# limanling/clip-event

Measured on AMD Instinct MI355X. Metric: image-text pairs/sec/GPU, ViT-B/32 224px x 77-tok, global-batch contrastive, higher is better.
Workload: dtype bf16; 1 GPU; ViT-B/32 224px x 77-tok, bf16 operands, per-GPU batch 256, K=1, InfoNCE only, full train step (fwd+bwd+clip_grad_norm+Adam), random-init weights; global_batch=256, parallelism=dp1, captions=SOT + U[8,75] random ids + EOT, zero-padded to 77 (SURVEY 8(d) c2), text_rows=live tokens SOT..EOT only: 54.8% of B*77 rows (identical results, see DESIGN.md), fresh_captions_every_step=True, alignment=False, cu_hog=0, nt_pgrid=256, full=False

## Files before the change

### clip_event_amd/csrc/attention.hip

```cpp
#include <map>
#include <mutex>

#include <type_traits>

#include "common.hpp"
#include "../../include/clip_event_hip.h"

namespace {

constexpr int HD = 64;
constexpr int ROW = 160;

typedef __attribute__((address_space(3))) s16x4 lds_s16x4;
typedef __attribute__((ext_vector_type(8))) short s16x8;

__device__ __forceinline__ bf16x8 tr_pair(const char* p0, const char* p1) {
    s16x4 lo = __builtin_amdgcn_ds_read_tr16_b64_v4i16((lds_s16x4*)p0);
    s16x4 hi = __builtin_amdgcn_ds_read_tr16_b64_v4i16((lds_s16x4*)p1);
    s16x8 v = {lo[0], lo[1], lo[2], lo[3], hi[0], hi[1], hi[2], hi[3]};
    return __builtin_bit_cast(bf16x8, v);
}

__device__ __forceinline__ bf16x8 pack8(const f32x4& a, const f32x4& b) {
    u32x4 v = {pack_bf2(a[0], a[1]), pack_bf2(a[2], a[3]), pack_bf2(b[0], b[1]), pack_bf2(b[2], b[3])};
// ... 113 lines not shown
                *reinterpret_cast<u32x2*>(orow + ct * 16) = pk;
            }
            if (g == 0) lse[((long)b * H + h) * Lmax + i] = mx + __logf(sum);
        }
    }
}

template <int T>
__global__ __launch_bounds__(512) void attn_bwd_kernel(const bf16_t* __restrict__ qkv, long ld,
                                                       const bf16_t* __restrict__ o, long ldo,
                                                       const bf16_t* __restrict__ dout, long lddo,
                                                       const float* __restrict__ lse, bf16_t* __restrict__ dqkv,
                                                       long lddq, float* __restrict__ bias_grad,
                                                       const int* __restrict__ cu, int Lmax, int H, int D,
                                                       int causal, float scale) {
    extern __shared__ __attribute__((aligned(16))) char smem[];
    constexpr int Lp = T * 16;
    constexpr int PROW = Lp * 2 + 32;
    char* sA = smem;
    char* sB = sA + Lp * ROW;
    char* sP = sB + Lp * ROW;
    char* sDS = sP + Lp * PROW;
    auto csum = [&](int i) __attribute__((always_inline)) -> float* { return reinterpret_cast<float*>(sP + (i >> 3) * PROW + Lp * 2 + (i & 7) * 4); };
    const int tid = threadIdx.x, lane = tid & 63;
    const int wave = __builtin_amdgcn_readfirstlane(tid >> 6), nw = blockDim.x >> 6;
    const int b = blockIdx.x / H, h = blockIdx.x - b * H;
    const long row0 = cu ? (long)cu[b] : (long)b * Lmax;
    const int L = cu ? min(cu[b + 1] - cu[b], Lmax) : Lmax;
    if (L <= 0) return;
    const int Tl = ((L + 31) >> 5) << 1;
    const int Ll = Tl * 16;
    const bf16_t* base = qkv + row0 * ld + h * HD;
    const bf16_t* dob = dout + row0 * lddo + h * HD;
    const bf16_t* ob = o + row0 * ldo + h * HD;
    bf16_t* dbase = dqkv + row0 * lddq + h * HD;

    for (int i = tid; i < 192; i += blockDim.x) *csum(i) = 0.f;
    const int li = lane & 15, g = lane >> 4;
    u32x4 rK[2], rV[2], rQ[2], rD[2];
#pragma unroll
    for (int c = 0; c < 2; ++c) {
        const int idx = tid + c * blockDim.x;
        const int r = idx >> 3, ch = idx & 7;
        const u32x4 z = {0u, 0u, 0u, 0u};
        rK[c] = z; rV[c] = z; rQ[c] = z; rD[c] = z;
        if (idx < Ll * 8 && r < L) {
            rK[c] = *reinterpret_cast<const u32x4*>(base + D + (long)r * ld + ch * 8);
            rV[c] = *reinterpret_cast<const u32x4*>(base + 2 * D + (long)r * ld + ch * 8);
            rQ[c] = *reinterpret_cast<const u32x4*>(base + (long)r * ld + ch * 8);
            rD[c] = *reinterpret_cast<const u32x4*>(dob + (long)r * lddo + ch * 8);
        }
    }
    const int strip = wave;
    const bool has_strip = strip < Tl;
    const int i = strip * 16 + li;
    const bool iok = has_strip && i < L;
    const int iq = min(i, L - 1);
    float dl = 0.f, lsei = 0.f;
    bf16x8 qf[2], df[2];
    if (has_strip) {
        const u32x4* pd = reinterpret_cast<const u32x4*>(dob + (long)iq * lddo + g * 16);
        const u32x4* po = reinterpret_cast<const u32x4*>(ob + (long)iq * ldo + g * 16);
#pragma unroll
        for (int v = 0; v < 2; ++v) {
            u32x4 a = pd[v], c = po[v];
#pragma unroll
            for (int e = 0; e < 4; ++e) dl += bf_lo(a[e]) * bf_lo(c[e]) + bf_hi(a[e]) * bf_hi(c[e]);
        }
        lsei = lse[((long)b * H + h) * Lmax + iq];
#pragma unroll
        for (int ks = 0; ks < 2; ++ks) {
            qf[ks] = *reinterpret_cast<const bf16x8*>(base + (long)iq * ld + ks * 32 + g * 8);
            df[ks] = *reinterpret_cast<const bf16x8*>(dob + (long)iq * lddo + ks * 32 + g * 8);
        }
    }
#pragma unroll
    for (int c = 0; c < 2; ++c) {
        const int idx = tid + c * blockDim.x;
        if (idx < Ll * 8) {
            *reinterpret_cast<u32x4*>(sA + (idx >> 3) * ROW + (idx & 7) * 16) = rK[c];
            *reinterpret_cast<u32x4*>(sB + (idx >> 3) * ROW + (idx & 7) * 16) = rV[c];
        }
    }
    __syncthreads();
    dl += __shfl_xor(dl, 16, 64);
    dl += __shfl_xor(dl, 32, 64);

    if (has_strip) {
        f32x4 p[T], ds[T];
#pragma unroll
        for (int t = 0; t < T; ++t) {
            p[t] = f32x4{0.f, 0.f, 0.f, 0.f};
            ds[t] = f32x4{0.f, 0.f, 0.f, 0.f};
            if (t >= Tl) continue;
#pragma unroll
            for (int ks = 0; ks < 2; ++ks) {
                bf16x8 kf = *reinterpret_cast<const bf16x8*>(sA + (t * 16 + li) * ROW + (ks * 4 + g) * 16);
                bf16x8 vf = *reinterpret_cast<const bf16x8*>(sB + (t * 16 + li) * ROW + (ks * 4 + g) * 16);
                p[t] = __builtin_amdgcn_mfma_f32_16x16x32_bf16(kf, qf[ks], p[t], 0, 0, 0);
                ds[t] = __builtin_amdgcn_mfma_f32_16x16x32_bf16(vf, df[ks], ds[t], 0, 0, 0);
            }
#pragma unroll
            for (int r = 0; r < 4; ++r) {
                const int j = t * 16 + g * 4 + r;
                const bool ok = iok && (j < L) && (!causal || j <= i);
                const float pv = ok ? __expf(p[t][r] * scale - lsei) : 0.f;
                p[t][r] = pv;
                ds[t][r] = pv * (ds[t][r] - dl) * scale;
            }
            u32x2 pk = {pack_bf2(p[t][0], p[t][1]), pack_bf2(p[t][2], p[t][3])};
            u32x2 dk = {pack_bf2(ds[t][0], ds[t][1]), pack_bf2(ds[t][2], ds[t][3])};
            *reinterpret_cast<u32x2*>(sP + i * PROW + (t * 16 + g * 4) * 2) = pk;
            *reinterpret_cast<u32x2*>(sDS + i * PROW + (t * 16 + g * 4) * 2) = dk;
        }
        f32x4 acc[4];
#pragma unroll
        for (int ct = 0; ct < 4; ++ct) acc[ct] = f32x4{0.f, 0.f, 0.f, 0.f};
#pragma unroll
        for (int sidx = 0; sidx < T / 2; ++sidx) {
            if (2 * sidx >= Tl) continue;
            bf16x8 sf = pack8(ds[2 * sidx], ds[2 * sidx + 1]);
            const char* krow = sA + (32 * sidx + 4 * g + (li >> 2)) * ROW + (4 * (li & 3)) * 2;
#pragma unroll
            for (int ct = 0; ct < 4; ++ct) {
                bf16x8 kf = tr_pair(krow + ct * 32, krow + ct * 32 + 16 * ROW);
                acc[ct] = __builtin_amdgcn_mfma_f32_16x16x32_bf16(kf, sf, acc[ct], 0, 0, 0);
            }
        }
        if (iok) {
            bf16_t* qrow = dbase + (long)i * lddq + 4 * g;
#pragma unroll
            for (int ct = 0; ct < 4; ++ct) {
                u32x2 pk = {pack_bf2(acc[ct][0], acc[ct][1]), pack_bf2(acc[ct][2], acc[ct][3])};
                *reinterpret_cast<u32x2*>(qrow + ct * 16) = pk;
            }
        }
        if (bias_grad) {
            float vals[16];
#pragma unroll
            for (int ct = 0; ct < 4; ++ct)
#pragma unroll
                for (int r = 0; r < 4; ++r) vals[ct * 4 + r] = acc[ct][r];
// ... 37 lines not shown
                av[ct] = __builtin_amdgcn_mfma_f32_16x16x32_bf16(dof, pf, av[ct], 0, 0, 0);
                ak[ct] = __builtin_amdgcn_mfma_f32_16x16x32_bf16(qf, sf, ak[ct], 0, 0, 0);
            }
        }
        if (j < L) {
            bf16_t* krow = dbase + (long)j * lddq + D + 4 * g;
            bf16_t* vrow = dbase + (long)j * lddq + 2 * D + 4 * g;
#pragma unroll
            for (int ct = 0; ct < 4; ++ct) {
                u32x2 pk = {pack_bf2(ak[ct][0], ak[ct][1]), pack_bf2(ak[ct][2], ak[ct][3])};
                u32x2 pv = {pack_bf2(av[ct][0], av[ct][1]), pack_bf2(av[ct][2], av[ct][3])};
                *reinterpret_cast<u32x2*>(krow + ct * 16) = pk;
                *reinterpret_cast<u32x2*>(vrow + ct * 16) = pv;
            }
        }
        if (bias_grad) {
            float vk[16], vv[16];
#pragma unroll
            for (int ct = 0; ct < 4; ++ct)
#pragma unroll
                for (int r = 0; r < 4; ++r) {
                    vk[ct * 4 + r] = ak[ct][r];
                    vv[ct * 4 + r] = av[ct][r];
                }
            const float tk = row16_colsum(vk, li), tv = row16_colsum(vv, li);
            const int k = row16_colsum_index(li);
            atomicAdd(csum(64 + (k >> 2) * 16 + 4 * g + (k & 3)), tk);
            atomicAdd(csum(128 + (k >> 2) * 16 + 4 * g + (k & 3)), tv);
        }
    }
    if (bias_grad) {
        __syncthreads();
        for (int i = tid; i < 192; i += blockDim.x) atomicAdd(bias_grad + (i >> 6) * D + h * HD + (i & 63), *csum(i));
    }
}

constexpr int LB = 64;
constexpr int LPROW = LB * 2 + 32;

__device__ __forceinline__ void stage_block(char* dst, const bf16_t* src, long ld, int row0, int L, int tid) {
#pragma unroll
    for (int c = 0; c < 2; ++c) {
        const int idx = tid + c * 256;
        const int r = idx >> 3, ch = idx & 7;
        u32x4 v = {0u, 0u, 0u, 0u};
        if (row0 + r < L) v = *reinterpret_cast<const u32x4*>(src + (long)(row0 + r) * ld + ch * 8);
        *reinterpret_cast<u32x4*>(dst + r * ROW + ch * 16) = v;
    }
}

struct BlockRegs { u32x4 v[2]; };
__device__ __forceinline__ BlockRegs load_block(const bf16_t* src, long ld, int row0, int L, int tid) {
    BlockRegs b;
#pragma unroll
    for (int c = 0; c < 2; ++c) {
        const int idx = tid + c * 256;
        const int r = idx >> 3, ch = idx & 7;
        b.v[c] = u32x4{0u, 0u, 0u, 0u};
        if (row0 + r < L) b.v[c] = *reinterpret_cast<const u32x4*>(src + (long)(row0 + r) * ld + ch * 8);
    }
    return b;
}
__device__ __forceinline__ void store_block(char* dst, const BlockRegs& b, int tid) {
#pragma unroll
    for (int c = 0; c < 2; ++c) {
        const int idx = tid + c * 256;
// ... 562 lines not shown
        if (nk == 1)
            hipLaunchKernelGGL(attn_bwd_long_dkv_kernel<1>, grid1, dim3(256), 0, sl, (const bf16_t*)qkv, ld, (const bf16_t*)o, ldo,
                               (const bf16_t*)dout, lddo, lse, (bf16_t*)dqkv, lddq, bias_grad, delta, L, H, D, causal, 0.125f, attn_xcd_order());
        else
            hipLaunchKernelGGL(attn_bwd_long_dkv_kernel<2>, grid2, dim3(256), 0, sl, (const bf16_t*)qkv, ld, (const bf16_t*)o, ldo,
                               (const bf16_t*)dout, lddo, lse, (bf16_t*)dqkv, lddq, bias_grad, delta, L, H, D, causal, 0.125f, attn_xcd_order());
        CE_LAUNCH_CHECK();
        return 0;
    }
    const int T = tiles_for(L);
    const int Lp = T * 16;
    int nw = T;
    if (nw > 8) nw = 8;
    const size_t lds = 2 * (size_t)Lp * ROW + 2 * (size_t)Lp * (Lp * 2 + 32);
    const float scale = 0.125f;
    hipStream_t s = (hipStream_t)stream;
    CeProfScope prof(CE_PROF_ATTN_BWD, 10.0 * B * H * (double)L * L * HD, 2.0 * (double)B * L * (8.0 * D), s);
#define CALL(TT)                                                                                                   \
    do {                                                                                                           \
        static std::once_flag attr;                                                                                \
        std::call_once(attr, [] {                                                                                  \
            hipFuncSetAttribute(reinterpret_cast<const void*>(attn_bwd_kernel<TT>),                                \
                                hipFuncAttributeMaxDynamicSharedMemorySize, 160 * 1024);                           \
        });                                                                                                        \
        hipLaunchKernelGGL(attn_bwd_kernel<TT>, dim3(B * H), dim3(64 * nw), lds, s, (const bf16_t*)qkv, ld,        \
                           (const bf16_t*)o, ldo, (const bf16_t*)dout, lddo, lse, (bf16_t*)dqkv, lddq, bias_grad, cu_seqlens, L, \
                           H, D, causal, scale);                                                                           \
    } while (0)
    ATTN_DISPATCH(T, CALL);
#undef CALL
    CE_LAUNCH_CHECK();
    return 0;
}
```

### clip_event_amd/csrc/tower.cpp

```cpp
#include <hip/hip_runtime.h>
#include <stdlib.h>

#include <map>
#include <mutex>

#include "common.hpp"
#include "tn_plan.hpp"
#include "../../include/clip_event_hip.h"

namespace {

constexpr int WG_MAX_BLOCKS = TN_GROUP_MAX_BLOCKS;
constexpr int WG_SETS = WG_MAX_BLOCKS + 1;
constexpr int LNP_RING = 8;

struct Carver {
    char* base;
    size_t off = 0;
    explicit Carver(void* b) : base(reinterpret_cast<char*>(b)) {}
    template <typename T>
    T* take(size_t n) {
        off = (off + 255) & ~size_t(255);
        T* p = base ? reinterpret_cast<T*>(base + off) : nullptr;
        off += n * sizeof(T);
// ... 96 lines not shown
    CE_CHECK_ARG(rows > 0 && (long)rows <= (long)batch * d->tokens, "tower: rows=%d outside 1..batch*tokens", rows);
    CE_CHECK_ARG(cu || rows == batch * d->tokens, "tower: a dense batch has batch*tokens rows (got %d)", rows);
    return 0;
}

int check_desc(const ce_tower_desc* d, int batch) {
    CE_CHECK_ARG(d && d->blocks, "tower: null descriptor");
    CE_CHECK_ARG(d->layers > 0 && d->layers <= Layout::MAX_LAYERS, "tower: layers=%d out of range", d->layers);
    CE_CHECK_ARG(d->width == d->heads * 64, "tower: width %d != heads %d * 64", d->width, d->heads);
    CE_CHECK_ARG(d->tokens > 0 && d->tokens <= 4096, "tower: tokens=%d unsupported (1..4096)", d->tokens);
    CE_CHECK_ARG(batch > 0, "tower: empty batch");
    CE_CHECK_ARG(d->stream16 == 0 || d->stream16 == 1, "tower: stream16=%d (0: fp32 residual stream, 1: fp16)", d->stream16);
    return 0;
}

#define TRY(call)            \
    do {                     \
        int rc__ = (call);   \
        if (rc__ != 0) return rc__; \
    } while (0)

int linear(bool use8, const Layout& L, const void*& q8_of, const void* A, long lda, const void* W, const void* W8, const float* S8, int M,
           int N, int K, int epi, const float* bias, const void* resid, long ldr, void* out, long ldo, void* out2,
           long ldo2, const void* aux, long ldaux, void* stream) {
    if (use8 && W8 && S8 && K % 128 == 0 && K <= 4096) {
        if (q8_of != A || lda != K) TRY(ce_quant_rows_fp8(A, lda, L.q8, K, L.q8s, M, K, stream));
        q8_of = nullptr;
        return ce_gemm_nt_fp8(L.q8, K, L.q8s, W8, K, S8, M, N, K, epi, bias, resid, ldr, out, ldo, out2, ldo2, aux, ldaux,
                              stream);
    }
    return ce_gemm_nt(A, lda, W, K, M, N, K, epi, bias, resid, ldr, out, ldo, out2, ldo2, aux, ldaux, stream);
}

int forward_run(const ce_tower_desc* d, int batch, int rows, const int* cu_seqlens, const void* x0, Layout& L, void* x_out,
                const int* sel_rows, bool infer, void* stream) {
    const int M = rows, w = d->width;
    const bool f8 = (d->fp8 & 1) != 0;
    const int ST = d->stream16 ? CE_T_F16 : CE_T_F32;
    const int EPI_RESID = d->stream16 ? CE_EPI_BIAS_RESID_F16 : CE_EPI_BIAS_RESID_F32;
    const int EPI_FC = infer ? CE_EPI_BIAS_QGELU_BF16 : CE_EPI_BIAS_GELU;
    const long esz = d->stream16 ? 2 : 4;
    const void* x = x0;
    const void* q8_of = nullptr;
    const bool lnq = f8 && w % 128 == 0 && w <= 4096;
    for (int l = 0; l < d->layers; ++l) {
        const ce_block_params& p = d->blocks[l];
        BlockStash& s = L.blk[l];
        void* xo = (l + 1 < d->layers) ? s.x_out : x_out;
        TRY(ce_layernorm_fwd_q8(x, ST, w, nullptr, p.ln1_w, p.ln1_b, s.h1, CE_T_BF16, w, s.mean1, s.rstd1, M, w, 1e-5f,
                                lnq ? L.q8 : nullptr, w, L.q8s, stream));
        if (lnq) q8_of = s.h1;
        TRY(linear(f8, L, q8_of, s.h1, w, p.w_qkv, p.w8_qkv, p.s8_qkv, M, 3 * w, w, CE_EPI_BIAS_BF16, p.b_qkv, nullptr, 0, s.qkv, 3 * w, nullptr, 0,
                       nullptr, 0, stream));
        TRY(ce_attention_fwd(s.qkv, 3 * w, s.o, w, s.lse, cu_seqlens, batch, d->tokens, d->heads, d->causal, stream));
        if (sel_rows && l + 1 == d->layers) {
            const int Bn = batch;
            TRY(ce_copy_rows(s.o, w * 2L, sel_rows, L.os, w * 2L, nullptr, Bn, w * 2, stream));
            TRY(ce_copy_rows(x, w * esz, sel_rows, L.xs_in, w * esz, nullptr, Bn, (int)(w * esz), stream));
            TRY(linear(f8, L, q8_of, L.os, w, p.w_out, p.w8_out, p.s8_out, Bn, w, w, EPI_RESID, p.b_out, L.xs_in, w, L.xs_mid, w, nullptr,
                           0, nullptr, 0, stream));
            TRY(ce_layernorm_fwd_t(L.xs_mid, ST, w, nullptr, p.ln2_w, p.ln2_b, L.h2s, CE_T_BF16, w, L.means, L.rstds, Bn, w, 1e-5f, stream));
            TRY(linear(f8, L, q8_of, L.h2s, w, p.w_fc, p.w8_fc, p.s8_fc, Bn, 4 * w, w, EPI_FC, p.b_fc, nullptr, 0, infer ? L.gs : L.as, 4 * w,
                           infer ? nullptr : L.gs, infer ? 0 : 4 * w, nullptr, 0, stream));
            TRY(linear(f8, L, q8_of, L.gs, 4 * w, p.w_proj, p.w8_proj, p.s8_proj, Bn, w, 4 * w, EPI_RESID, p.b_proj, L.xs_mid, w, x_out, w,
                           nullptr, 0, nullptr, 0, stream));
            break;
        }
        TRY(linear(f8, L, q8_of, s.o, w, p.w_out, p.w8_out, p.s8_out, M, w, w, EPI_RESID, p.b_out, x, w, s.x_mid, w, nullptr, 0, nullptr,
                       0, stream));
        TRY(ce_layernorm_fwd_q8(s.x_mid, ST, w, nullptr, p.ln2_w, p.ln2_b, s.h2, CE_T_BF16, w, s.mean2, s.rstd2, M, w, 1e-5f,
                                lnq ? L.q8 : nullptr, w, L.q8s, stream));
        if (lnq) q8_of = s.h2;
        TRY(linear(f8, L, q8_of, s.h2, w, p.w_fc, p.w8_fc, p.s8_fc, M, 4 * w, w, EPI_FC, p.b_fc, nullptr, 0, infer ? s.g : s.a, 4 * w,
                       infer ? nullptr : s.g, infer ? 0 : 4 * w, nullptr, 0, stream));
        TRY(linear(f8, L, q8_of, s.g, 4 * w, p.w_proj, p.w8_proj, p.s8_proj, M, w, 4 * w, EPI_RESID, p.b_proj, s.x_mid, w, xo, w,
                       nullptr, 0, nullptr, 0, stream));
        x = xo;
    }
    return 0;
}

}

extern "C" size_t ce_tower_workspace_bytes(const ce_tower_desc* d, int batch) {
    if (check_desc(d, batch) != 0) return 0;
    Layout L;
    carve(d, batch, (size_t)batch * d->tokens, nullptr, L);
    return L.bytes;
}

// ... 90 lines not shown
    } pend;
    auto queue = [&](const void* P, long ldp, const void* Q, long ldq, int Nn, int Kk, float* out, long ldo) {
        const int i = pend.count++;
        pend.P[i] = P; pend.ldp[i] = ldp; pend.Q[i] = Q; pend.ldq[i] = ldq;
        pend.Nn[i] = Nn; pend.Kk[i] = Kk; pend.out[i] = out; pend.ldo[i] = ldo;
    };
    auto flush = [&]() -> int {
        if (pend.count == 0) return 0;
        const int rc = ce_gemm_tn_grouped_ex(pend.count, pend.P, pend.ldp, pend.Q, pend.ldq, M, pend.Nn, pend.Kk, pend.out,
                                             pend.ldo, 0, d->wgrad_overwrite, stream);
        pend.count = 0;
        pend.blocks = 0;
        return rc;
    };
    int top = layer_hi;
    if (layer_hi < last) {
    } else if (sel_rows) {
        CE_CHECK_ARG(dx_sel, "ce_tower_backward: pruned mode needs dx_sel");
        const int l = top, Bn = batch, q = l % WG_SETS;
        const ce_block_params& p = d->blocks[l];
        BlockStash& s = L.blk[l];
        const void* x_in = (l == 0) ? x0 : L.blk[l - 1].x_out;
        TRY(ce_cast_bf16(dx_sel, L.dxbs, (long)Bn * w, stream));
        TRY(linear(b8, L, q8_of, L.dxbs, w, p.wt_proj, p.wt8_proj, p.st8_proj, Bn, 4 * w, w, CE_EPI_GELUGRAD_BF16, nullptr, nullptr, 0, L.das, 4 * w, nullptr,
                       0, L.as, 4 * w, stream));
        TRY(ce_colsum_bf16(L.dxbs, w, p.g_b_proj, Bn, w, stream));
        TRY(linear(b8, L, q8_of, L.das, 4 * w, p.wt_fc, p.wt8_fc, p.st8_fc, Bn, w, 4 * w, CE_EPI_BF16, nullptr, nullptr, 0, L.dhs, w, nullptr, 0,
                       nullptr, 0, stream));
        TRY(ce_colsum_bf16(L.das, 4 * w, p.g_b_fc, Bn, 4 * w, stream));
        TRY(ce_layernorm_bwd_t(L.dhs, CE_T_BF16, w, L.xs_mid, ST, w, nullptr, L.means, L.rstds, p.ln2_w, dx_sel, CE_T_F32, L.dxs_mid,
                               ST, w, L.dxb2s, w, p.g_ln2_w, p.g_ln2_b, p.g_b_out, GS, Bn, w, stream));
        TRY(linear(b8, L, q8_of, L.dxb2s, w, p.wt_out, p.wt8_out, p.st8_out, Bn, w, w, CE_EPI_BF16, nullptr, nullptr, 0, L.dos, w, nullptr, 0, nullptr, 0,
                       stream));
        TRY(ce_scatter_rows_zero(L.dos, w * 2L, L.d_o, w * 2L, sel_rows, Bn, M, w * 2, stream));
        TRY(ce_attention_bwd(s.qkv, 3 * w, s.o, w, L.d_o, w, s.lse, L.dqkv[q], 3 * w, p.g_b_qkv, cu_seqlens, batch, d->tokens, d->heads,
                             d->causal, stream));
        {
            const void* P[3] = {L.dxbs, L.das, L.dxb2s};
            const long ldp[3] = {w, 4L * w, w};
            const void* Q[3] = {L.gs, L.h2s, L.os};
            const long ldq[3] = {4L * w, w, w};
            const int Nn[3] = {w, 4 * w, w};
            const int Kk[3] = {4 * w, w, w};
            float* out[3] = {p.g_w_proj, p.g_w_fc, p.g_w_out};
            const long ldo[3] = {4L * w, w, w};
            TRY(ce_gemm_tn_grouped_ex(3, P, ldp, Q, ldq, Bn, Nn, Kk, out, ldo, 0, d->wgrad_overwrite, stream));
        }
        queue(L.dqkv[q], 3L * w, s.h1, w, 3 * w, w, p.g_w_qkv, w);
        TRY(linear(b8, L, q8_of, L.dqkv[q], 3 * w, p.wt_qkv, p.wt8_qkv, p.st8_qkv, M, w, 3 * w, CE_EPI_BF16, nullptr, nullptr, 0, L.dh, w, nullptr, 0,
                       nullptr, 0, stream));
        TRY(ce_scatter_rows_zero(L.dxs_mid, w * esz, dx, w * esz, sel_rows, Bn, M, (int)(w * esz), stream));
        TRY(ce_layernorm_bwd_t(L.dh, CE_T_BF16, w, x_in, ST, w, nullptr, s.mean1, s.rstd1, p.ln1_w, dx, ST, dx, ST, w,
                               L.dxb[(l + WG_SETS - 1) % WG_SETS], w, p.g_ln1_w, p.g_ln1_b,
                               (l > 0) ? d->blocks[l - 1].g_b_proj : nullptr, GS, M, w, stream));
        top = l - 1;
    } else {
        if (d->stream16) TRY(ce_cast_scaled(dx, ST, L.dxb[top % WG_SETS], CE_T_BF16, GS, 1, (long)M * w, stream));
        else TRY(ce_cast_bf16(reinterpret_cast<const float*>(dx), L.dxb[top % WG_SETS], (long)M * w, stream));
    }
    plan_cuts(top, layer_lo, pend.count > 0 ? 3 * tn_problem_tiles(M, w, w) : 0);
    for (int l = top; l >= layer_lo; --l) {
        const ce_block_params& p = d->blocks[l];
        BlockStash& s = L.blk[l];
        const int q = l % WG_SETS;
        bf16_t *dxb_a = L.dxb[q], *dxb_b = L.dxb2[q], *da = L.da[q], *dqkv = L.dqkv[q];
        const void* x_in = (l == 0) ? x0 : L.blk[l - 1].x_out;
        TRY(linear(b8, L, q8_of, dxb_a, w, p.wt_proj, p.wt8_proj, p.st8_proj, M, 4 * w, w, CE_EPI_GELUGRAD_BF16, nullptr, nullptr, 0, da, 4 * w, p.g_b_fc,
                       4 * w, s.a, 4 * w, stream));
        if (l == last) TRY(ce_colsum_bf16(dxb_a, w, p.g_b_proj, M, w, stream));
// ... 31 lines not shown
```

### clip_event_amd/ops.py

```python
from __future__ import annotations

from typing import Optional

import torch

from . import _lib as L
from ._lib import check, lib, ptr, stream


def _rows(t: torch.Tensor) -> int:
    return t.shape[0]


def _nt_tail(epilogue, bias, resid, out, out2, ldo2, aux):
    return (epilogue, ptr(bias), ptr(resid), resid.stride(0) if resid is not None else 0, ptr(out), out.stride(0), ptr(out2),
            ldo2, ptr(aux), aux.stride(0) if aux is not None else 0, stream())


def gemm_nt(a: torch.Tensor, b: torch.Tensor, epilogue: int, *, bias=None, resid=None, out=None, out2=None,
            aux=None, M: Optional[int] = None) -> torch.Tensor:
    assert a.dtype == torch.bfloat16 and b.dtype == torch.bfloat16 and a.is_cuda and b.is_cuda
    M = a.shape[0] if M is None else M
    K = a.shape[1]
    N = b.shape[0]
# ... 80 lines not shown
    return buf[:1]


def cast_scaled(x: torch.Tensor, dtype, scale: torch.Tensor, divide: bool = False):
    y = torch.empty_like(x, dtype=dtype)
    check(lib().ce_cast_scaled(ptr(x), _TYPE[x.dtype], ptr(y), _TYPE[dtype], ptr(scale), 1 if divide else 0,
                               x.numel(), stream()), "ce_cast_scaled")
    return y


def cast_t(x: torch.Tensor, dtype, mul: float = 1.0):
    y = torch.empty_like(x, dtype=dtype)
    check(lib().ce_cast_t(ptr(x), _TYPE[x.dtype], ptr(y), _TYPE[dtype], mul, x.numel(), stream()),
          "ce_cast_t")
    return y


def attention_fwd(qkv: torch.Tensor, B: int, L: int, H: int, causal: bool, cu_seqlens=None):
    assert qkv.dtype == torch.bfloat16
    o = torch.empty(qkv.shape[0], H * 64, device=qkv.device, dtype=torch.bfloat16)
    lse = torch.empty(B * H * L, device=qkv.device, dtype=torch.float32)
    check(lib().ce_attention_fwd(ptr(qkv), qkv.stride(0), ptr(o), o.stride(0), ptr(lse),
                                 ptr(cu_seqlens), B, L, H, 1 if causal else 0, stream()),
          "ce_attention_fwd")
    return o, lse


def attention_bwd(qkv, o, dout, lse, B: int, L: int, H: int, causal: bool, bias_grad=None, cu_seqlens=None):
    dqkv = torch.empty_like(qkv)
    check(lib().ce_attention_bwd(ptr(qkv), qkv.stride(0), ptr(o), o.stride(0), ptr(dout),
                                 dout.stride(0), ptr(lse), ptr(dqkv), dqkv.stride(0), ptr(bias_grad),
                                 ptr(cu_seqlens), B, L, H, 1 if causal else 0, stream()),
          "ce_attention_bwd")
    return dqkv


def probe_mfma(shape: int, a_frags: torch.Tensor, b_frags: torch.Tensor) -> torch.Tensor:
    out = torch.empty(64, 4 if shape == 16 else 16, device=a_frags.device, dtype=torch.float32)
    check(lib().ce_probe_mfma(shape, ptr(a_frags), ptr(b_frags), ptr(out), stream()), "ce_probe_mfma")
    return out


def probe_tr16(image: torch.Tensor, byte_off: torch.Tensor) -> torch.Tensor:
    out = torch.empty(64, 4, device=image.device, dtype=torch.int16)
    check(lib().ce_probe_tr16(ptr(image), image.numel(), ptr(byte_off), ptr(out), stream()), "ce_probe_tr16")
    return out


def quant_rows_fp8(x: torch.Tensor):
    assert x.dtype == torch.bfloat16 and x.is_cuda and x.stride(1) == 1
    M, K = x.shape
    q = torch.empty(M, K, dtype=torch.uint8, device=x.device)
    scale = torch.empty(M, dtype=torch.float32, device=x.device)
    check(lib().ce_quant_rows_fp8(ptr(x), x.stride(0), ptr(q), K, ptr(scale), M, K, stream()),
          "ce_quant_rows_fp8")
    return q, scale


def gemm_nt_fp8(a8, sa, b8, sb, epilogue: int, *, bias=None, resid=None, aux=None, colsum=None):
    M, K = a8.shape
    N = b8.shape[0]
    f32_out = epilogue == L.EPI_BIAS_RESID_F32
    out = torch.empty(M, N, device=a8.device, dtype=torch.float32 if f32_out else torch.bfloat16)
    out2 = torch.empty_like(out) if epilogue == L.EPI_BIAS_GELU else colsum
    ldo2 = out2.stride(0) if epilogue == L.EPI_BIAS_GELU else 0
    check(lib().ce_gemm_nt_fp8(ptr(a8), a8.stride(0), ptr(sa), ptr(b8), b8.stride(0), ptr(sb), M, N, K,
# ... 47 lines not shown
```

### include/clip_event_hip.h

```cpp
#ifndef CLIP_EVENT_HIP_H
#define CLIP_EVENT_HIP_H

#include <stddef.h>
#include <stdint.h>

#ifdef __cplusplus
extern "C" {
#endif

const char* ce_last_error(void);
int ce_version(void);

enum {
    CE_EPI_BF16 = 0,
    CE_EPI_F32 = 1,
    CE_EPI_BIAS_BF16 = 2,
    CE_EPI_BIAS_F32 = 3,
    CE_EPI_BIAS_RESID_F32 = 4,
    CE_EPI_BIAS_GELU = 5,
    CE_EPI_GELUGRAD_BF16 = 6,
    CE_EPI_BIAS_RESID_F16 = 7,
    CE_EPI_BIAS_QGELU_BF16 = 8
};

// ... 46 lines not shown
int ce_layernorm_bwd(const void* dy, long lddy, int dy_f32, const float* x, long ldx, const int* rows,
                     const float* mean, const float* rstd, const float* w, const float* dx_in, float* dx_out,
                     long lddx, void* dxb, long lddxb, float* dw, float* db, float* dxsum, int M, int D,
                     void* stream);
int ce_layernorm_bwd_t(const void* dy, int dy_type, long lddy, const void* x, int x_type, long ldx, const int* rows,
                       const float* mean, const float* rstd, const float* w, const void* dx_in, int dxin_type,
                       void* dx_out, int dx_type, long lddx, void* dxb, long lddxb, float* dw, float* db, float* dxsum,
                       const float* gscale, int M, int D, void* stream);

int ce_layernorm_bwd_q8(const void* dy, int dy_type, long lddy, const void* x, int x_type, long ldx, const int* rows,
                        const float* mean, const float* rstd, const float* w, const void* dx_in, int dxin_type,
                        void* dx_out, int dx_type, long lddx, void* dxb, long lddxb, float* dw, float* db, float* dxsum,
                        const float* gscale, int M, int D, void* q8, long ldq, float* qscale, void* stream);

int ce_layernorm_bwd_blocks(int M, int D);
int ce_layernorm_bwd_partials(const void* dy, int dy_type, long lddy, const void* x, int x_type, long ldx, const int* rows,
                              const float* mean, const float* rstd, const float* w, const void* dx_in, int dxin_type,
                              void* dx_out, int dx_type, long lddx, void* dxb, long lddxb, int want_dxsum,
                              const float* gscale, int M, int D, void* q8, long ldq, float* qscale, float* partials,
                              void* stream);
#define CE_LN_FOLD_MAX 64
typedef struct ce_ln_fold_job {
    const float* partials;
    float *dw, *db, *dxsum;
    int blocks, D;
} ce_ln_fold_job;
int ce_layernorm_fold(const ce_ln_fold_job* jobs , int njobs, void* stream);

int ce_attention_fwd(const void* qkv, long ld, void* o, long ldo, float* lse, const int* cu_seqlens, int B, int L,
                     int H, int causal, void* stream);
int ce_attention_bwd(const void* qkv, long ld, const void* o, long ldo, const void* dout, long lddo,
                     const float* lse, void* dqkv, long lddq, float* bias_grad, const int* cu_seqlens, int B, int L,
                     int H, int causal, void* stream);

int ce_im2col(const float* image, void* patches, int B, int resolution, int patch, int k_padded, void* stream);
int ce_vision_assemble(const float* patch_out, const float* cls, const float* pos, float* x0, int B, int tokens,
                       int D, void* stream);
int ce_vision_assemble_bwd(const float* dx0, void* dpatch, int B, int tokens, int D, void* stream);
int ce_patch_keep(long seed, long draw, long sample0, int B, int N, int keep, int* keep_idx, int* inv, void* stream);
int ce_im2col_rows(const float* image, const int* keep_idx, void* patches, int B, int keep, int resolution, int patch,
                   int k_padded, void* stream);
int ce_vision_assemble_rows(const float* patch_out, const int* keep_idx, const float* cls, const float* pos, float* x0,
                            int B, int N, int keep, int D, void* stream);
int ce_pos_embed_bwd_rows(const float* dx0, const int* inv, float* dpos, int B, int N, int keep, int D, void* stream);
int ce_token_embed(const int64_t* ids, const int* src_rows, const float* table, const float* pos, float* x0, long rows,
                   int tokens, int D, int vocab, void* stream);
int ce_token_embed_t(const int64_t* ids, const int* src_rows, const float* table, const float* pos, void* x0, int x0_type,
                     long rows, int tokens, int D, int vocab, void* stream);
int ce_token_embed_bwd(const int64_t* ids, const int* src_rows, const float* dx0, float* dtable, long rows, int D,
                       int vocab, void* stream);
int ce_pos_embed_bwd_packed(const float* dx0, const int* cu_seqlens, float* dpos, int n, int tokens, int D,
                            void* stream);
int ce_batch_reduce(const float* x, float* out, int B, long slab, long n, int accumulate, void* stream);
int ce_colsum_bf16(const void* x, long ld, float* out, int M, int N, void* stream);
int ce_cast_transpose(const float* w, void* w16, long ld16, void* w16t, long ld16t, int R, int C, void* stream);
int ce_cast_bf16(const float* x, void* y, long n, void* stream);
int ce_cast_t(const void* x, int src_type, void* y, int dst_type, float mul, long n, void* stream);
int ce_cast_scaled(const void* x, int src_type, void* y, int dst_type, const float* scale, int divide, long n, void* stream);
#define CE_GRAD_SCALE_SCRATCH 256
int ce_grad_scale(const float* x, long n, float target, float* scratch, float* scale, void* stream);
int ce_stream16_set_counters(unsigned int* device_counters);
int ce_add_cols(const float* src, long lds, float* dst, long ldd, int rows, int cols, void* stream);
int ce_copy_rows(const void* src, long src_stride_bytes, const int* src_rows, void* dst, long dst_stride_bytes,
                 const int* dst_rows, int n, int row_bytes, void* stream);
int ce_scatter_rows_zero(const void* src, long src_stride_bytes, void* dst, long dst_stride_bytes, const int* dst_rows, int n,
                         int M, int row_bytes, void* stream);
// ... 277 lines not shown
```

Measured before the change: 20950 pairs/s (whole job).

## Compute last-layer attention only for selected rows in forward and backward

In the final transformer layer only the pooled row (CLS or EOT) per sequence is consumed, so new single-query attention kernels compute forward output and LSE for just that row, and a matching backward kernel produces dQ/dK/dV and bias grads from the selected row's gradient. This replaces full-sequence attention plus the row gather and scatter-zero steps. The existing backward kernel also now computes the softmax-gradient correction term from P·dP instead of reading O, which removes the O load. It adds new kernels with atomics for bias grads and an env switch (on by default), and relies on the pruned-row dqkv zeroing being correct.

```diff
diff --git a/clip_event_amd/csrc/attention.hip b/clip_event_amd/csrc/attention.hip
--- a/clip_event_amd/csrc/attention.hip
+++ b/clip_event_amd/csrc/attention.hip
@@ -169,7 +169,7 @@
     const int Ll = Tl * 16;
     const bf16_t* base = qkv + row0 * ld + h * HD;
     const bf16_t* dob = dout + row0 * lddo + h * HD;
-    const bf16_t* ob = o + row0 * ldo + h * HD;
+    (void)o; (void)ldo;
     bf16_t* dbase = dqkv + row0 * lddq + h * HD;
 
     for (int i = tid; i < 192; i += blockDim.x) *csum(i) = 0.f;
@@ -193,17 +193,9 @@
     const int i = strip * 16 + li;
     const bool iok = has_strip && i < L;
     const int iq = min(i, L - 1);
-    float dl = 0.f, lsei = 0.f;
+    float lsei = 0.f;
     bf16x8 qf[2], df[2];
     if (has_strip) {
-        const u32x4* pd = reinterpret_cast<const u32x4*>(dob + (long)iq * lddo + g * 16);
-        const u32x4* po = reinterpret_cast<const u32x4*>(ob + (long)iq * ldo + g * 16);
-#pragma unroll
-        for (int v = 0; v < 2; ++v) {
-            u32x4 a = pd[v], c = po[v];
-#pragma unroll
-            for (int e = 0; e < 4; ++e) dl += bf_lo(a[e]) * bf_lo(c[e]) + bf_hi(a[e]) * bf_hi(c[e]);
-        }
         lsei = lse[((long)b * H + h) * Lmax + iq];
 #pragma unroll
         for (int ks = 0; ks < 2; ++ks) {
@@ -220,11 +212,10 @@
         }
     }
     __syncthreads();
-    dl += __shfl_xor(dl, 16, 64);
-    dl += __shfl_xor(dl, 32, 64);
 
     if (has_strip) {
         f32x4 p[T], ds[T];
+        float dl = 0.f;
 #pragma unroll
         for (int t = 0; t < T; ++t) {
             p[t] = f32x4{0.f, 0.f, 0.f, 0.f};
@@ -243,8 +234,16 @@
                 const bool ok = iok && (j < L) && (!causal || j <= i);
                 const float pv = ok ? __expf(p[t][r] * scale - lsei) : 0.f;
                 p[t][r] = pv;
-                ds[t][r] = pv * (ds[t][r] - dl) * scale;
-            }
+                dl += pv * ds[t][r];
+            }
+        }
+        dl += __shfl_xor(dl, 16, 64);
+        dl += __shfl_xor(dl, 32, 64);
+#pragma unroll
+        for (int t = 0; t < T; ++t) {
+            if (t >= Tl) continue;
+#pragma unroll
+            for (int r = 0; r < 4; ++r) ds[t][r] = p[t][r] * (ds[t][r] - dl) * scale;
             u32x2 pk = {pack_bf2(p[t][0], p[t][1]), pack_bf2(p[t][2], p[t][3])};
             u32x2 dk = {pack_bf2(ds[t][0], ds[t][1]), pack_bf2(ds[t][2], ds[t][3])};
             *reinterpret_cast<u32x2*>(sP + i * PROW + (t * 16 + g * 4) * 2) = pk;
@@ -348,6 +347,196 @@
     if (bias_grad) {
         __syncthreads();
         for (int i = tid; i < 192; i += blockDim.x) atomicAdd(bias_grad + (i >> 6) * D + h * HD + (i & 63), *csum(i));
+    }
+}
+
+__device__ __forceinline__ void unpack8(const u32x4& raw, float (&f)[8]) {
+#pragma unroll
+    for (int e = 0; e < 4; ++e) {
+        f[2 * e] = bf_lo(raw[e]);
+        f[2 * e + 1] = bf_hi(raw[e]);
+    }
+}
+__device__ __forceinline__ u32x4 pack8f(const float (&f)[8]) {
+    return u32x4{pack_bf2(f[0], f[1]), pack_bf2(f[2], f[3]), pack_bf2(f[4], f[5]), pack_bf2(f[6], f[7])};
+}
+__device__ __forceinline__ float bf_round(float x) { return bf_lo(pack_bf2(x, 0.f)); }
+__device__ __forceinline__ float sum_over_c(float v) {
+    v += __shfl_xor(v, 1, 64);
+    v += __shfl_xor(v, 2, 64);
+    v += __shfl_xor(v, 4, 64);
+    return v;
+}
+__device__ __forceinline__ float sum_over_rr(float v) {
+    v += __shfl_xor(v, 8, 64);
+    v += __shfl_xor(v, 16, 64);
+    v += __shfl_xor(v, 32, 64);
+    return v;
+}
+
+__device__ __forceinline__ bool sel_coords(const int* __restrict__ cu, const int* __restrict__ sel, int b, int Lmax, int causal,
+                                           long& row0, int& L, int& is, int& n) {
+    row0 = cu ? (long)cu[b] : (long)b * Lmax;
+    L = cu ? min(cu[b + 1] - cu[b], Lmax) : Lmax;
+    if (L <= 0) return false;
+    const long rel = (long)sel[b] - row0;
+    if (rel < 0 || rel >= L) return false;
+    is = (int)rel;
+    n = causal ? is + 1 : L;
+    return true;
+}
+
+template <int NP>
+__device__ __forceinline__ void load_kv_sel(const bf16_t* base, int D, long ld, int n, int rr, int c, u32x4 (&kr)[NP], u32x4 (&vr)[NP]) {
+    const uint32_t span = (uint32_t)(((long)n - 1) * ld * 2 + HD * 2);
+    const __amdgpu_buffer_rsrc_t rK = make_rsrc(base + D, span), rV = make_rsrc(base + 2 * D, span);
+#pragma unroll
+    for (int pp = 0; pp < NP; ++pp) {
+        const int j = pp * 8 + rr;
+        const uint32_t off = j < n ? (uint32_t)(j * ld * 2 + c * 16) : 0x80000000u;
+        kr[pp] = __builtin_amdgcn_raw_buffer_load_b128(rK, off, 0, 0);
+        vr[pp] = __builtin_amdgcn_raw_buffer_load_b128(rV, off, 0, 0);
+    }
+}
+
+template <int NP>
+__global__ __launch_bounds__(64) void attn_fwd_sel_kernel(const bf16_t* __restrict__ qkv, long ld, const int* __restrict__ sel,
+                                                          bf16_t* __restrict__ o_sel, long ldo, float* __restrict__ lse_sel,
+                                                          const int* __restrict__ cu, int Lmax, int H, int D, int causal,
+                                                          float scale) {
+    const int lane = threadIdx.x, rr = lane >> 3, c = lane & 7;
+    const int b = blockIdx.x / H, h = blockIdx.x - b * H;
+    long row0;
+    int L, is, n;
+    if (!sel_coords(cu, sel, b, Lmax, causal, row0, L, is, n)) return;
+    const bf16_t* base = qkv + row0 * ld + h * HD;
+    const u32x4 qraw = *reinterpret_cast<const u32x4*>(base + (long)is * ld + c * 8);
+    u32x4 kr[NP], vr[NP];
+    load_kv_sel<NP>(base, D, ld, n, rr, c, kr, vr);
+    float q[8];
+    unpack8(qraw, q);
+    float s[NP];
+    float mx = -INFINITY;
+#pragma unroll
+    for (int pp = 0; pp < NP; ++pp) {
+        float k[8], dot = 0.f;
+        unpack8(kr[pp], k);
+#pragma unroll
+        for (int e = 0; e < 8; ++e) dot += q[e] * k[e];
+        dot = sum_over_c(dot);
+        s[pp] = (pp * 8 + rr < n) ? dot * scale : -INFINITY;
+        mx = fmaxf(mx, s[pp]);
+    }
+    mx = fmaxf(mx, __shfl_xor(mx, 8, 64));
+    mx = fmaxf(mx, __shfl_xor(mx, 16, 64));
+    mx = fmaxf(mx, __shfl_xor(mx, 32, 64));
+    float sum = 0.f, acc[8];
+#pragma unroll
+    for (int e = 0; e < 8; ++e) acc[e] = 0.f;
+#pragma unroll
+    for (int pp = 0; pp < NP; ++pp) {
+        const float pe = __expf(s[pp] - mx);
+        sum += pe;
+        const float pv = bf_round(pe);
+        float v[8];
+        unpack8(vr[pp], v);
+#pragma unroll
+        for (int e = 0; e < 8; ++e) acc[e] += pv * v[e];
+    }
+    sum = sum_over_rr(sum);
+#pragma unroll
+    for (int e = 0; e < 8; ++e) acc[e] = sum_over_rr(acc[e]);
+    if (rr == 0) {
+        const float inv = 1.0f / sum;
+#pragma unroll
+        for (int e = 0; e < 8; ++e) acc[e] *= inv;
+        *reinterpret_cast<u32x4*>(o_sel + (long)b * ldo + h * HD + c * 8) = pack8f(acc);
+    }
+    if (lane == 0) lse_sel[(long)b * H + h] = mx + __logf(sum);
+}
+
+template <int NP>
+__global__ __launch_bounds__(64) void attn_bwd_sel_kernel(const bf16_t* __restrict__ qkv, long ld, const int* __restrict__ sel,
+                                                          const bf16_t* __restrict__ dout_sel, long lddo,
+                                                          const float* __restrict__ lse_sel, bf16_t* __restrict__ dqkv, long lddq,
+                                                          float* __restrict__ bias_grad, const int* __restrict__ cu, int Lmax,
+                                                          int H, int D, int causal, float scale) {
+    const int lane = threadIdx.x, rr = lane >> 3, c = lane & 7;
+    const int b = blockIdx.x / H, h = blockIdx.x - b * H;
+    long row0;
+    int L, is, n;
+    if (!sel_coords(cu, sel, b, Lmax, causal, row0, L, is, n)) return;
+    const bf16_t* base = qkv + row0 * ld + h * HD;
+    bf16_t* dbase = dqkv + row0 * lddq + h * HD;
+    const u32x4 qraw = *reinterpret_cast<const u32x4*>(base + (long)is * ld + c * 8);
+    const u32x4 draw = *reinterpret_cast<const u32x4*>(dout_sel + (long)b * lddo + h * HD + c * 8);
+    const float lsev = lse_sel[(long)b * H + h];
+    u32x4 kr[NP], vr[NP];
+    load_kv_sel<NP>(base, D, ld, n, rr, c, kr, vr);
+    float q[8], dO[8];
+    unpack8(qraw, q);
+    unpack8(draw, dO);
+    float p[NP], dp[NP];
+    float dl = 0.f;
+#pragma unroll
+    for (int pp = 0; pp < NP; ++pp) {
+        float k[8], v[8], sd = 0.f, dd = 0.f;
+        unpack8(kr[pp], k);
+        unpack8(vr[pp], v);
+#pragma unroll
+        for (int e = 0; e < 8; ++e) {
+            sd += q[e] * k[e];
+            dd += dO[e] * v[e];
+        }
+        sd = sum_over_c(sd);
+        dp[pp] = sum_over_c(dd);
+        p[pp] = (pp * 8 + rr < n) ? __expf(sd * scale - lsev) : 0.f;
+        dl += p[pp] * dp[pp];
+    }
+    dl = sum_over_rr(dl);
+    float acc[8], sds = 0.f, sp = 0.f;
+#pragma unroll
+    for (int e = 0; e < 8; ++e) acc[e] = 0.f;
+    const u32x4 zero = {0u, 0u, 0u, 0u};
+#pragma unroll
+    for (int pp = 0; pp < NP; ++pp) {
+        const int j = pp * 8 + rr;
+        const float dsv = bf_round(p[pp] * (dp[pp] - dl) * scale), pb = bf_round(p[pp]);
+        float k[8], gk[8], gv[8];
+        unpack8(kr[pp], k);
+#pragma unroll
+        for (int e = 0; e < 8; ++e) {
+            acc[e] += dsv * k[e];
+            gk[e] = dsv * q[e];
+            gv[e] = pb * dO[e];
+        }
+        sds += dsv;
+        sp += pb;
+        if (j < L) {
+            bf16_t* row = dbase + (long)j * lddq + c * 8;
+            if (j != is) *reinterpret_cast<u32x4*>(row) = zero;
+            *reinterpret_cast<u32x4*>(row + D) = pack8f(gk);
+            *reinterpret_cast<u32x4*>(row + 2 * D) = pack8f(gv);
+        }
+    }
+#pragma unroll
+    for (int e = 0; e < 8; ++e) acc[e] = sum_over_rr(acc[e]);
+    if (rr == 0) *reinterpret_cast<u32x4*>(dbase + (long)is * lddq + c * 8) = pack8f(acc);
+    if (bias_grad) {
+        sds = sum_over_rr(sds);
+        sp = sum_over_rr(sp);
+        float aq = acc[0], aqq = q[0], ado = dO[0];
+#pragma unroll
+        for (int e = 1; e < 8; ++e)
+            if (rr == e) {
+                aq = acc[e];
+                aqq = q[e];
+                ado = dO[e];
+            }
+        float* col = bias_grad + h * HD + c * 8 + rr;
+        atomicAdd(col, aq);
+        atomicAdd(col + D, aqq * sds);
+        atomicAdd(col + 2 * D, ado * sp);
     }
 }
 
@@ -976,3 +1165,42 @@
     CE_LAUNCH_CHECK();
     return 0;
 }
+
+extern "C" int ce_attention_fwd_sel(const void* qkv, long ld, const int* sel_rows, void* o_sel, long ldo, float* lse_sel,
+                                    const int* cu_seqlens, int B, int L, int H, int causal, void* stream) {
+    CE_CHECK_ARG(B > 0 && L > 0 && H > 0, "ce_attention_fwd_sel: empty problem");
+    CE_CHECK_ARG(L <= 128, "ce_attention_fwd_sel: sequence length %d above 128", L);
+    CE_CHECK_ARG(qkv && sel_rows && o_sel && lse_sel, "ce_attention_fwd_sel: null buffer");
+    CE_CHECK_ARG(ld % 8 == 0 && ldo % 8 == 0, "ce_attention_fwd_sel: leading dimensions must be multiples of 8");
+    const int D = H * HD;
+    const int T = tiles_for(L);
+    hipStream_t s = (hipStream_t)stream;
+    CeProfScope prof(CE_PROF_ATTN_FWD, 4.0 * B * H * (double)L * HD, 2.0 * (double)B * L * (2.0 * D), s);
+#define CALL(TT)                                                                                                                \
+    hipLaunchKernelGGL(attn_fwd_sel_kernel<2 * TT>, dim3(B * H), dim3(64), 0, s, (const bf16_t*)qkv, ld, sel_rows, (bf16_t*)o_sel, \
+                       ldo, lse_sel, cu_seqlens, L, H, D, causal, 0.125f)
+    ATTN_DISPATCH(T, CALL);
+#undef CALL
+    CE_LAUNCH_CHECK();
+    return 0;
+}
+
+extern "C" int ce_attention_bwd_sel(const void* qkv, long ld, const int* sel_rows, const void* dout_sel, long lddo,
+                                    const float* lse_sel, void* dqkv, long lddq, float* bias_grad, const int* cu_seqlens, int B,
+                                    int L, int H, int causal, void* stream) {
+    CE_CHECK_ARG(B > 0 && L > 0 && H > 0, "ce_attention_bwd_sel: empty problem");
+    CE_CHECK_ARG(L <= 128, "ce_attention_bwd_sel: sequence length %d above 128", L);
+    CE_CHECK_ARG(qkv && sel_rows && dout_sel && lse_sel && dqkv, "ce_attention_bwd_sel: null buffer");
+    CE_CHECK_ARG(ld % 8 == 0 && lddo % 8 == 0 && lddq % 8 == 0, "ce_attention_bwd_sel: leading dimensions must be multiples of 8");
+    const int D = H * HD;
+    const int T = tiles_for(L);
+    hipStream_t s = (hipStream_t)stream;
+    CeProfScope prof(CE_PROF_ATTN_BWD, 10.0 * B * H * (double)L * HD, 2.0 * (double)B * L * (5.0 * D), s);
+#define CALL(TT)                                                                                                                \
+    hipLaunchKernelGGL(attn_bwd_sel_kernel<2 * TT>, dim3(B * H), dim3(64), 0, s, (const bf16_t*)qkv, ld, sel_rows,               \
+                       (const bf16_t*)dout_sel, lddo, lse_sel, (bf16_t*)dqkv, lddq, bias_grad, cu_seqlens, L, H, D, causal, 0.125f)
+    ATTN_DISPATCH(T, CALL);
+#undef CALL
+    CE_LAUNCH_CHECK();
+    return 0;
+}
diff --git a/clip_event_amd/csrc/tower.cpp b/clip_event_amd/csrc/tower.cpp
--- a/clip_event_amd/csrc/tower.cpp
+++ b/clip_event_amd/csrc/tower.cpp
@@ -152,6 +152,11 @@
     return ce_gemm_nt(A, lda, W, K, M, N, K, epi, bias, resid, ldr, out, ldo, out2, ldo2, aux, ldaux, stream);
 }
 
+bool attn_sel(const ce_tower_desc* d) {
+    static const int on = getenv("CE_ATTN_SEL") ? atoi(getenv("CE_ATTN_SEL")) : 1;
+    return on && d->tokens <= 128;
+}
+
 int forward_run(const ce_tower_desc* d, int batch, int rows, const int* cu_seqlens, const void* x0, Layout& L, void* x_out,
                 const int* sel_rows, bool infer, void* stream) {
     const int M = rows, w = d->width;
@@ -172,10 +177,15 @@
         if (lnq) q8_of = s.h1;
         TRY(linear(f8, L, q8_of, s.h1, w, p.w_qkv, p.w8_qkv, p.s8_qkv, M, 3 * w, w, CE_EPI_BIAS_BF16, p.b_qkv, nullptr, 0, s.qkv, 3 * w, nullptr, 0,
                        nullptr, 0, stream));
-        TRY(ce_attention_fwd(s.qkv, 3 * w, s.o, w, s.lse, cu_seqlens, batch, d->tokens, d->heads, d->causal, stream));
-        if (sel_rows && l + 1 == d->layers) {
+        const bool pruned = sel_rows && l + 1 == d->layers;
+        if (pruned && attn_sel(d)) {
+            TRY(ce_attention_fwd_sel(s.qkv, 3 * w, sel_rows, L.os, w, s.lse, cu_seqlens, batch, d->tokens, d->heads, d->causal, stream));
+        } else {
+            TRY(ce_attention_fwd(s.qkv, 3 * w, s.o, w, s.lse, cu_seqlens, batch, d->tokens, d->heads, d->causal, stream));
+        }
+        if (pruned) {
             const int Bn = batch;
-            TRY(ce_copy_rows(s.o, w * 2L, sel_rows, L.os, w * 2L, nullptr, Bn, w * 2, stream));
+            if (!attn_sel(d)) TRY(ce_copy_rows(s.o, w * 2L, sel_rows, L.os, w * 2L, nullptr, Bn, w * 2, stream));
             TRY(ce_copy_rows(x, w * esz, sel_rows, L.xs_in, w * esz, nullptr, Bn, (int)(w * esz), stream));
             TRY(linear(f8, L, q8_of, L.os, w, p.w_out, p.w8_out, p.s8_out, Bn, w, w, EPI_RESID, p.b_out, L.xs_in, w, L.xs_mid, w, nullptr,
                            0, nullptr, 0, stream));
@@ -332,9 +342,14 @@
                                ST, w, L.dxb2s, w, p.g_ln2_w, p.g_ln2_b, p.g_b_out, GS, Bn, w, stream));
         TRY(linear(b8, L, q8_of, L.dxb2s, w, p.wt_out, p.wt8_out, p.st8_out, Bn, w, w, CE_EPI_BF16, nullptr, nullptr, 0, L.dos, w, nullptr, 0, nullptr, 0,
                        stream));
-        TRY(ce_scatter_rows_zero(L.dos, w * 2L, L.d_o, w * 2L, sel_rows, Bn, M, w * 2, stream));
-        TRY(ce_attention_bwd(s.qkv, 3 * w, s.o, w, L.d_o, w, s.lse, L.dqkv[q], 3 * w, p.g_b_qkv, cu_seqlens, batch, d->tokens, d->heads,
-                             d->causal, stream));
+        if (attn_sel(d)) {
+            TRY(ce_attention_bwd_sel(s.qkv, 3 * w, sel_rows, L.dos, w, s.lse, L.dqkv[q], 3 * w, p.g_b_qkv, cu_seqlens, batch, d->tokens,
+                                     d->heads, d->causal, stream));
+        } else {
+            TRY(ce_scatter_rows_zero(L.dos, w * 2L, L.d_o, w * 2L, sel_rows, Bn, M, w * 2, stream));
+            TRY(ce_attention_bwd(s.qkv, 3 * w, s.o, w, L.d_o, w, s.lse, L.dqkv[q], 3 * w, p.g_b_qkv, cu_seqlens, batch, d->tokens, d->heads,
+                                 d->causal, stream));
+        }
         {
             const void* P[3] = {L.dxbs, L.das, L.dxb2s};
             const long ldp[3] = {w, 4L * w, w};
diff --git a/clip_event_amd/ops.py b/clip_event_amd/ops.py
--- a/clip_event_amd/ops.py
+++ b/clip_event_amd/ops.py
@@ -136,6 +136,25 @@
                                  dout.stride(0), ptr(lse), ptr(dqkv), dqkv.stride(0), ptr(bias_grad),
                                  ptr(cu_seqlens), B, L, H, 1 if causal else 0, stream()),
           "ce_attention_bwd")
+    return dqkv
+
+
+def attention_fwd_sel(qkv: torch.Tensor, sel_rows: torch.Tensor, B: int, L: int, H: int, causal: bool, cu_seqlens=None):
+    assert qkv.dtype == torch.bfloat16 and sel_rows.dtype == torch.int32
+    o = torch.empty(B, H * 64, device=qkv.device, dtype=torch.bfloat16)
+    lse = torch.empty(B * H, device=qkv.device, dtype=torch.float32)
+    check(lib().ce_attention_fwd_sel(ptr(qkv), qkv.stride(0), ptr(sel_rows), ptr(o), o.stride(0), ptr(lse),
+                                     ptr(cu_seqlens), B, L, H, 1 if causal else 0, stream()),
+          "ce_attention_fwd_sel")
+    return o, lse
+
+
+def attention_bwd_sel(qkv, sel_rows, dout_sel, lse_sel, B: int, L: int, H: int, causal: bool, bias_grad=None, cu_seqlens=None):
+    dqkv = torch.empty_like(qkv)
+    check(lib().ce_attention_bwd_sel(ptr(qkv), qkv.stride(0), ptr(sel_rows), ptr(dout_sel), dout_sel.stride(0), ptr(lse_sel),
+                                     ptr(dqkv), dqkv.stride(0), ptr(bias_grad), ptr(cu_seqlens), B, L, H,
+                                     1 if causal else 0, stream()),
+          "ce_attention_bwd_sel")
     return dqkv
 
 
diff --git a/include/clip_event_hip.h b/include/clip_event_hip.h
--- a/include/clip_event_hip.h
+++ b/include/clip_event_hip.h
@@ -102,6 +102,11 @@
 int ce_attention_bwd(const void* qkv, long ld, const void* o, long ldo, const void* dout, long lddo,
                      const float* lse, void* dqkv, long lddq, float* bias_grad, const int* cu_seqlens, int B, int L,
                      int H, int causal, void* stream);
+int ce_attention_fwd_sel(const void* qkv, long ld, const int* sel_rows, void* o_sel, long ldo, float* lse_sel,
+                         const int* cu_seqlens, int B, int L, int H, int causal, void* stream);
+int ce_attention_bwd_sel(const void* qkv, long ld, const int* sel_rows, const void* dout_sel, long lddo,
+                         const float* lse_sel, void* dqkv, long lddq, float* bias_grad, const int* cu_seqlens, int B,
+                         int L, int H, int causal, void* stream);
 
 int ce_im2col(const float* image, void* patches, int B, int resolution, int patch, int k_padded, void* stream);
 int ce_vision_assemble(const float* patch_out, const float* cls, const float* pos, float* x0, int B, int tokens,
```

After: 21130 pairs/s (whole job), median of 6. No clear change (+0.9%).
